# aleflabo/PREGO

Hardware: AMD Instinct MI355X
Metric: frames/sec (per-frame action logits) on Assembly101-O TSN features (higher is better)
Workload: dtype fp16; 1 GPU; BASELINE configs[1]: Assembly101-O-test-split-shaped eval set, MiniROAD eval path (rgb+flow fp32 [T,2048] each -> per-frame probs[86] + argmax); clips_per_gpu=182, frames_per_gpu=2306143, min_T=3342, max_T=33981, flow=non-zero (full K=4096 layer1 GEMM), parallelism=clip-sharded dp1, no collective: every rank its own eval-set-sized clip list, weights=random init, seed 20

## Files before the change

### prego_amd/csrc/ff_pass.hip

```cpp
#include "common.h"
#include "kernels.h"
#include "gemm_tile.h"
#include "pass_handshake.h"

#define FF_TIMEOUT_TICKS 200000000ull

__device__ __forceinline__ bool ffp_wait_ge(const unsigned* p, unsigned need, unsigned* abort_word, unsigned code) {
  if (__hip_atomic_load(p, __ATOMIC_RELAXED, __HIP_MEMORY_SCOPE_AGENT) >= need) return true;
  const unsigned long long t0 = __builtin_amdgcn_s_memrealtime();
  unsigned spins = 0;
  for (;;) {
    __builtin_amdgcn_s_sleep(8);
    if (__hip_atomic_load(p, __ATOMIC_RELAXED, __HIP_MEMORY_SCOPE_AGENT) >= need) return true;
    if ((++spins & 31u) == 0u) {
      if (__hip_atomic_load(abort_word, __ATOMIC_RELAXED, __HIP_MEMORY_SCOPE_AGENT)) return false;
      if (__builtin_amdgcn_s_memrealtime() - t0 > FF_TIMEOUT_TICKS) {
        __hip_atomic_store(abort_word, code, __ATOMIC_RELAXED, __HIP_MEMORY_SCOPE_AGENT);
        return false;
      }
    }
  }
}

template <typename OT, bool SC1OUT>
__device__ __forceinline__ void ffp_tile(char* smem, const bf16_t* __restrict__ A, int lda, int rows, const bf16_t* __restrict__ B, int ldb,
                                         const float* __restrict__ bias, bf16_t* __restrict__ C, int ldc, int K) {
  int tid = threadIdx.x;
  asm volatile("" : "+v"(tid));
  const int lane = tid & 63;
  const int wave = __builtin_amdgcn_readfirstlane(tid >> 6);
  const int grp = wave >> 2, wc = wave & 3;
  int a_off[2], b_off[2];
  pp_lane_offsets<false>(wave, lane, lda, ldb, 0, 0, a_off, b_off);
  const __amdgpu_buffer_rsrc_t rs_a = __builtin_amdgcn_make_buffer_rsrc((void*)A, 0, rows * lda * 2, 0x00020000);
  const __amdgpu_buffer_rsrc_t rs_b = __builtin_amdgcn_make_buffer_rsrc((void*)B, 0, 256 * ldb * 2, 0x00020000);
  const int fr = lane & 15, fq = lane >> 4;
  f32x4 acc[2][2][4][2];
#pragma unroll
  for (int x = 0; x < 2; ++x)
#pragma unroll
    for (int y = 0; y < 2; ++y)
#pragma unroll
      for (int i = 0; i < 4; ++i)
#pragma unroll
        for (int j = 0; j < 2; ++j) acc[x][y][i][j] = (f32x4){0.f, 0.f, 0.f, 0.f};
  pp_tile_loop<OT, false>((lds_char*)smem, rs_a, rs_b, a_off, b_off, lda, ldb, K / kPpBK, wave, lane, acc);
  float4 bv[2][2];
#pragma unroll
  for (int y = 0; y < 2; ++y)
#pragma unroll
    for (int j = 0; j < 2; ++j) bv[y][j] = *(const float4*)(bias + y * 128 + wc * 32 + fq * 8 + j * 4);
  const __amdgpu_buffer_rsrc_t rs_c = __builtin_amdgcn_make_buffer_rsrc((void*)C, 0, rows * ldc * 2, 0x00020000);
#pragma unroll
  for (int x = 0; x < 2; ++x)
#pragma unroll
    for (int y = 0; y < 2; ++y) {
      const int n = y * 128 + wc * 32 + fq * 8;
#pragma unroll
      for (int i = 0; i < 4; ++i) {
        const int m = x * 128 + grp * 64 + i * 16 + fr;
        const f32x4 v0 = acc[x][y][i][0], v1 = acc[x][y][i][1];
        u32x4 pk;
        pk[0] = op16<OT>::pack2_sat(v0[0] + bv[y][0].x, v0[1] + bv[y][0].y); pk[1] = op16<OT>::pack2_sat(v0[2] + bv[y][0].z, v0[3] + bv[y][0].w);
        pk[2] = op16<OT>::pack2_sat(v1[0] + bv[y][1].x, v1[1] + bv[y][1].y); pk[3] = op16<OT>::pack2_sat(v1[2] + bv[y][1].z, v1[3] + bv[y][1].w);
        if constexpr (SC1OUT) __builtin_amdgcn_raw_buffer_store_b128(pk, rs_c, (m * ldc + n) * 2, 0, AUX_SC1);
        else __builtin_amdgcn_raw_buffer_store_b128(pk, rs_c, (m * ldc + n) * 2, 0, 0);
      }
    }
}

template <typename OT, bool IN16>
__device__ __forceinline__ void ffp_pack_rows(const FfPassArgs& a, int my_rows, int wave, int lane, const char* srgb, const char* sflow,
                                              bf16_t* __restrict__ Xs) {
  constexpr int ES = IN16 ? 2 : 4, NV = IN16 ? 1 : 2;
  constexpr int PR = 2;
  const int din = a.kx;
  const int cr_rgb = (a.d_rgb + 2047) >> 11, cpr = cr_rgb + ((a.d_flow + 2047) >> 11);
  const int n_rounds = my_rows > 0 ? ((my_rows + PR - 1) / PR) * cpr : 0;
  auto readlane_ptr = [](const char* p, int l) -> const char* {
    const unsigned long long v = (unsigned long long)p;
    const unsigned lo = (unsigned)__builtin_amdgcn_readlane((int)(unsigned)v, l), hi = (unsigned)__builtin_amdgcn_readlane((int)(unsigned)(v >> 32), l);
// ... 287 lines not shown
#pragma unroll
      for (int e = 0; e < NR; ++e)
#pragma unroll
        for (int i = 0; i < MAXV; ++i)
          if (i < nv) raw[e][i] = nxt[e][i];
    }
  }
}

template <typename OT>
__device__ __forceinline__ void ffp_ln_any(const FfPassArgs& a, int nrows, const bf16_t* __restrict__ Ys, bf16_t* __restrict__ Es, const float* gb) {
  switch (a.E >> 9) {
    case 4: ffp_ln<OT, 4, 2>(a, nrows, Ys, Es, gb); break;
    case 2: ffp_ln<OT, 2, 4>(a, nrows, Ys, Es, gb); break;
    case 1: ffp_ln<OT, 1, 4>(a, nrows, Ys, Es, gb); break;
    default: ffp_ln_generic<OT, 8, 2>(a, nrows, Ys, Es); break;
  }
}

template <typename OT>
__global__ __launch_bounds__(512, 2) void ff_pass_kernel(FfPassArgs a) {
  extern __shared__ __attribute__((aligned(16))) char smem[];
  __shared__ int s_job[2];
  const int tid = threadIdx.x;
  const int xcc = __builtin_amdgcn_readfirstlane(__builtin_amdgcn_s_getreg((3 << 11) | 20) & 7);
  if (xcc < a.xcd_lo) return;
  if (tid == 0) {
    const unsigned nth = __hip_atomic_fetch_add(a.hs.ff_here + xcc, 1u, __ATOMIC_RELAXED, __HIP_MEMORY_SCOPE_AGENT);
    s_job[1] = hs_wait(a.hs, a.hs.ticks_all) == PREGO_HS_GO ? 1 : 0;
    if (a.max_wg > 0 && (int)nth >= a.max_wg) s_job[1] = 0;
  }
  __syncthreads();
  if (!__builtin_amdgcn_readfirstlane(s_job[1])) return;
  __shared__ __attribute__((aligned(16))) float s_gb[2 * FLN_MAX_E];
  if (a.E <= FLN_MAX_E)
    for (int c = tid; c < a.E; c += 512) { s_gb[c] = a.ln_g[c]; s_gb[FLN_MAX_E + c] = a.ln_b[c]; }
  const int q = xcc - a.xcd_lo, nf = 8 - a.xcd_lo;
  const int n_q = a.n_units > q ? (a.n_units - q + nf - 1) / nf : 0;
  const int sg = a.sg, tpr = sg * (2 + a.nt1 + a.nt2);
  const int n_rounds = (n_q + sg - 1) / sg + a.lag3;
  __shared__ unsigned long long s_stat[11];
  const bool stats = a.stats != nullptr && tid == 0;
  if (stats) {
    for (int e = 0; e < 8; ++e) s_stat[e] = 0;
    s_stat[9] = __builtin_amdgcn_s_memrealtime(); s_stat[8] = s_stat[9]; s_stat[10] = __builtin_amdgcn_s_memtime();
  }
#define FSTAT(i) do { if (stats) { const unsigned long long n_ = __builtin_amdgcn_s_memrealtime(); s_stat[i] += n_ - s_stat[8]; s_stat[8] = n_; } } while (0)
  for (;;) {
    __syncthreads();
    if (tid == 0) s_job[0] = (int)__hip_atomic_fetch_add(a.tick + q, 1u, __ATOMIC_RELAXED, __HIP_MEMORY_SCOPE_AGENT);
    __syncthreads();
    const int k = __builtin_amdgcn_readfirstlane(s_job[0]);
    const int round = k / tpr, j = k - round * tpr;
    FSTAT(5);
    if (round >= n_rounds) break;
    int type, i, nb = 0;
    if (j < sg) { type = 0; i = round * sg + j; }
    else if (j < sg + sg * a.nt1) { const int jj = j - sg; type = 1; nb = jj / sg; i = (round - a.lag1) * sg + (jj - nb * sg); }
    else if (j < 2 * sg + sg * a.nt1) { type = 2; i = (round - a.lag2) * sg + (j - sg - sg * a.nt1); }
    else { const int jj = j - 2 * sg - sg * a.nt1; type = 3; nb = jj / sg; i = (round - a.lag3) * sg + (jj - nb * sg); }
    if (i < 0 || i >= n_q) continue;
    const int u = q + i * nf;
    if (tid == 0) {
      bool ok = true;
      const int up = u - a.ring_units;
      if (type == 0) {
        if (up >= 0) ok = ffp_wait_ge(a.l1_cnt + up, (unsigned)a.nt1, a.abort_word, 0x100u);
      } else if (type == 1) {
        ok = ffp_wait_ge(a.pack_done + u, 1u, a.abort_word, 0x101u);
        if (ok && up >= 0) ok = ffp_wait_ge(a.ln_done + up, 1u, a.abort_word, 0x102u);
      } else if (type == 2) {
        ok = ffp_wait_ge(a.l1_cnt + u, (unsigned)a.nt1, a.abort_word, 0x103u);
        if (ok && up >= 0) ok = ffp_wait_ge(a.wih_cnt + up, (unsigned)a.nt2, a.abort_word, 0x104u);
      } else {
        ok = ffp_wait_ge(a.ln_done + u, 1u, a.abort_word, 0x105u);
        const int ug = u - a.gi_ring_units;
        if (ok && ug >= 0) ok = ffp_wait_ge(a.rec_cnt + (ug >> a.chunk_unit_shift), (unsigned)a.rec_expect, a.abort_word, 0x106u);
      }
      s_job[1] = ok ? 1 : 0;
    }
    __syncthreads();
    if (!__builtin_amdgcn_readfirstlane(s_job[1])) break;
    FSTAT(4);
    asm volatile("buffer_inv sc0" ::: "memory");
    const int row0 = u * 256;
    const int nrows = a.total_rows - row0 < 256 ? a.total_rows - row0 : 256;
    const size_t slot = (size_t)(u % a.ring_units) * 256;
    if (type == 0) {
      if (!(a.dbg & 1)) ffp_pack<OT>(a, row0, nrows, a.X + slot * a.kx);
    } else if (type == 1) {
      if (!(a.dbg & 4))
      ffp_tile<OT, false>(smem, a.X + slot * a.kx, a.kx, nrows, a.w1 + (size_t)nb * 256 * a.ld_w1, a.ld_w1, a.b1 + nb * 256,
                          a.Y + slot * a.E + nb * 256, a.E, a.kx);
    } else if (type == 2) {
      if (a.dbg & 2) { }
      else ffp_ln_any<OT>(a, nrows, a.Y + slot * a.E, a.Eb + slot * a.E, s_gb);
    } else {
      const size_t gslot = (size_t)(u & (a.gi_ring_units - 1)) * 256;
      if (!(a.dbg & 8))
      ffp_tile<OT, true>(smem, a.Eb + slot * a.E, a.E, nrows, a.w_ih + (size_t)nb * 256 * a.E, a.E, a.bias2 + nb * 256,
                         a.GI + gslot * a.n3 + nb * 256, a.n3, a.E);
    }
    asm volatile("s_waitcnt vmcnt(0)" ::: "memory");
    __syncthreads();
    FSTAT(type);
    if (tid == 0) {
      if (type == 0) __hip_atomic_store(a.pack_done + u, 1u, __ATOMIC_RELAXED, __HIP_MEMORY_SCOPE_AGENT);
      else if (type == 1) __hip_atomic_fetch_add(a.l1_cnt + u, 1u, __ATOMIC_RELAXED, __HIP_MEMORY_SCOPE_AGENT);
      else if (type == 2) __hip_atomic_store(a.ln_done + u, 1u, __ATOMIC_RELAXED, __HIP_MEMORY_SCOPE_AGENT);
      else {
        const unsigned old = __hip_atomic_fetch_add(a.wih_cnt + u, 1u, __ATOMIC_RELAXED, __HIP_MEMORY_SCOPE_AGENT);
        if (old + 1u == (unsigned)a.nt2)
          __hip_atomic_fetch_add(a.gi_cnt + (u >> a.chunk_unit_shift), 1u, __ATOMIC_RELAXED, __HIP_MEMORY_SCOPE_AGENT);
      }
    }
  }
  if (stats) {
    s_stat[7] = __builtin_amdgcn_s_memrealtime() - s_stat[9];
    s_stat[6] = __builtin_amdgcn_s_memtime() - s_stat[10];
    for (int e = 0; e < 8; ++e) atomicAdd(a.stats + e, s_stat[e]);
  }
#undef FSTAT
}

int launch_ff_pass(const FfPassArgs& a, hipStream_t s) {
  if (a.E % 512 || a.E > 4096 || a.kx % kPpBK || a.kx < 2 * kPpBK || a.n3 % 256 || a.xcd_lo < 1 || a.xcd_lo > 7) return -1;
  if (a.sg < 1 || a.ring_units % (8 - a.xcd_lo) || (a.gi_ring_units & (a.gi_ring_units - 1)) || a.nt1 != a.E / 256 || a.nt2 != a.n3 / 256) return -1;
  static DeviceOnce once;
  once.run([&] {
    (void)hipFuncSetAttribute((const void*)ff_pass_kernel<bf16_t>, hipFuncAttributeMaxDynamicSharedMemorySize, 2 * kPpBuf);
    (void)hipFuncSetAttribute((const void*)ff_pass_kernel<f16_t>, hipFuncAttributeMaxDynamicSharedMemorySize, 2 * kPpBuf);
  });
  if (a.f16) ff_pass_kernel<f16_t><<<256, 512, 2 * kPpBuf, s>>>(a);
  else ff_pass_kernel<bf16_t><<<256, 512, 2 * kPpBuf, s>>>(a);
  return 0;
}
```

### prego_amd/csrc/gemm_tile.h

```cpp
#pragma once
#include "common.h"
#include "kernels.h"
#include <type_traits>

template <typename F>
inline void gemm_epi_dispatch(int mode, bool f16, F&& f) {
  auto by_type = [&](auto e) { if (f16) f(e, f16_t{}); else f(e, bf16_t{}); };
  switch (mode) {
    case EPI_STORE: by_type(std::integral_constant<int, EPI_STORE>{}); break;
    case EPI_STORE_BF16: by_type(std::integral_constant<int, EPI_STORE_BF16>{}); break;
    case EPI_RESIDUAL: by_type(std::integral_constant<int, EPI_RESIDUAL>{}); break;
    case EPI_GELU_BF16: by_type(std::integral_constant<int, EPI_GELU_BF16>{}); break;
    case EPI_TOKENS: by_type(std::integral_constant<int, EPI_TOKENS>{}); break;
    default: by_type(std::integral_constant<int, EPI_QKV>{}); break;
  }
}

__device__ __forceinline__ int xcd_remap(int bid, int nwg) {
  const int q = nwg >> 3, r = nwg & 7, x = bid & 7;
  return (x < r ? x * (q + 1) : r * (q + 1) + (x - r) * q) + (bid >> 3);
}

__device__ __forceinline__ int tile_key_a(int r) { return (r >> 1) & 7; }
__device__ __forceinline__ int tile_key_b_perm(int r) { return ((r >> 1) & 1) | (((r >> 3) & 3) << 1); }
// ... 12 lines not shown
#pragma unroll
  for (int i = 0; i < 2; ++i) {
    const int r = (wave * 2 + i) * 8 + sr;
    const int c = scp ^ tile_key_a(r);
    const int cb = scp ^ tile_key_b_perm(r);
    if constexpr (SPLIT) {
      a_off[i] = r * lda * 2 + (c < 4 ? c * 16 : a_lo * 2 + (c - 4) * 16);
      b_off[i] = r * ldb * 2 + (cb < 4 ? cb * 16 : b_lo * 2 + (cb - 4) * 16);
    } else {
      a_off[i] = r * lda * 2 + c * 16;
      b_off[i] = r * ldb * 2 + cb * 16;
    }
  }
}

template <typename OT, bool SPLIT>
__device__ __forceinline__ void pp_tile_loop(lds_char* smem, __amdgpu_buffer_rsrc_t rs_a, __amdgpu_buffer_rsrc_t rs_b, const int (&a_off)[2],
                                             const int (&b_off)[2], int lda, int ldb, int nk, int wave, int lane, f32x4 (&acc)[2][2][4][2]) {
  const int grp = wave >> 2, wc = wave & 3;
  auto stage_a = [&](int hf, int kt) {
    lds_char* dst = smem + (kt & 1) * kPpBuf + hf * kPpHalf + wave * 2048;
    const int so = hf * 128 * lda * 2 + kt * (SPLIT ? kPpBK : kPpBK * 2);
#pragma unroll
    for (int i = 0; i < 2; ++i)
      __builtin_amdgcn_raw_ptr_buffer_load_lds(rs_a, (__attribute__((address_space(3))) void*)(dst + i * 1024), 16, a_off[i], so, 0, 0);
  };
  auto stage_b = [&](int hf, int kt) {
    lds_char* dst = smem + (kt & 1) * kPpBuf + (2 + hf) * kPpHalf + wave * 2048;
    const int so = hf * 128 * ldb * 2 + kt * (SPLIT ? kPpBK : kPpBK * 2);
#pragma unroll
    for (int i = 0; i < 2; ++i)
      __builtin_amdgcn_raw_ptr_buffer_load_lds(rs_b, (__attribute__((address_space(3))) void*)(dst + i * 1024), 16, b_off[i], so, 0, 0);
  };

  const int fr = lane & 15, fq = lane >> 4;
  bf16x8 a0[2][4], a1[2][4], b0[2][2], b1[2][2];
  auto read_a = [&](bf16x8 (&af)[2][4], int slot, int kt) {
    const lds_char* base = smem + (kt & 1) * kPpBuf + slot * kPpHalf;
#pragma unroll
    for (int ks = 0; ks < 2; ++ks)
#pragma unroll
      for (int i = 0; i < 4; ++i) {
        const int r = grp * 64 + fr;
        af[ks][i] = *(const lds_bf16x8*)(base + r * 128 + (((ks * 4 + fq) ^ tile_key_a(r)) << 4) + i * 2048);
      }
  };
  auto read_b = [&](bf16x8 (&bf)[2][2], int slot, int kt) {
    const lds_char* base = smem + (kt & 1) * kPpBuf + slot * kPpHalf;
// ... 26 lines not shown
      for (int ks = 0; ks < 2; ++ks)
#pragma unroll
        for (int i = 0; i < 4; ++i)
#pragma unroll
          for (int j = 0; j < 2; ++j) c[i][j] = op16<OT>::mfma(bf[ks][j], af[ks][i], c[i][j]);
    }
    __builtin_amdgcn_s_setprio(0);
    __builtin_amdgcn_sched_barrier(0);
  };
  auto bar = [&]() {
    __builtin_amdgcn_sched_barrier(0);
    __builtin_amdgcn_s_barrier();
    __builtin_amdgcn_sched_barrier(0);
  };

  stage_a(0, 0); stage_b(0, 0); stage_b(1, 0); stage_a(1, 0);
  stage_a(0, 1); stage_b(0, 1); stage_b(1, 1);
  GEMM_VMCNT(10);
  bar();
  read_a(a0, 0, 0);
  if (grp == 1) bar();
  for (int kt = 0; kt < nk; ++kt) {
    const bool full = kt + 2 < nk;
    read_b(b0, 2, kt);
    if (kt + 1 < nk) stage_a(1, kt + 1);
    if (full) GEMM_VMCNT(10); else GEMM_VMCNT(0);
    bar();
    mma(acc[0][0], a0, b0);
    bar();
    read_b(b1, 3, kt);
    if (full) { stage_a(0, kt + 2); GEMM_VMCNT(10); } else GEMM_VMCNT(0);
    bar();
// ... 88 lines not shown
```

### prego_amd/csrc/kernels.h

```cpp
#pragma once
#include <hip/hip_runtime_api.h>
#include <stddef.h>
#include <stdint.h>
#include <mutex>

const char* prego_tune_env(const char* name);

struct DeviceOnce {
  std::mutex mu;
  bool done[64] = {};
  template <class F> int run(F&& f) {
    int dev = 0;
    (void)hipGetDevice(&dev);
    if (dev < 0 || dev >= 64) { f(); return 0; }
    std::lock_guard<std::mutex> g(mu);
    if (!done[dev]) { f(); done[dev] = true; }
    return dev;
  }
};

#ifndef PREGO_HAVE_SLOTPLAN
struct SlotPlan {
  const int* rowoff; const int* nact; const int* seg_off; const int* seg_clip; const int* seg_start; const int* blk_step;
  int s_max; int n_slots;
// ... 59 lines not shown
  int E, n3;
  unsigned short* X; unsigned short* Y; unsigned short* Eb;
  unsigned short* GI;
  int ring_units, gi_ring_units;
  int total_rows, n_units;
  int xcd_lo;
  int chunk_unit_shift;
  int rec_expect;
  int nt1, nt2;
  int sg;
  int max_wg;
  int lag1, lag2, lag3;
  int dbg;
  unsigned long long* stats;
  int f16;
  unsigned* tick;
  unsigned* pack_done; unsigned* l1_cnt; unsigned* ln_done; unsigned* wih_cnt;
  unsigned* gi_cnt;
  const unsigned* rec_cnt;
  unsigned* abort_word;
  PassHandshake hs;
};
int launch_ff_pass(const FfPassArgs& a, hipStream_t s);
int launch_gru_recurrence_pass(int hid, GruArgs a, hipStream_t s);
int gru_group_size(bool bf16, int hid);
bool gru_hidden_supported(bool bf16, int hid);

struct GruArm { unsigned* hx; unsigned long long words_per_buf; unsigned pattern; unsigned* sync; };
GruArm gru_arm_desc(bool bf16, int hid, int G, void* hx, unsigned* sync);
void launch_gru_arm(const GruArm& arm, hipStream_t s);

// ... 402 lines not shown
```

### prego_amd/csrc/miniroad_split.cpp

```cpp
#include "miniroad_handle.h"

#include <algorithm>
#include <chrono>
#include <cstdlib>
#include <mutex>
#include <thread>

static int tuned_pow2(const char* name, int dflt) {
  const char* v = prego_tune_env(name);
  const int x = v ? atoi(v) : 0;
  return (x >= 16 && (x & (x - 1)) == 0) ? x : dflt;
}
static int split_gi_ring_units(int R) { return tuned_pow2("PREGO_SPLIT_GI_RING", R <= 3 ? 32 : 256); }
static const int kSplitRingPerXcd = (prego_tune_env("PREGO_SPLIT_RING_PER_XCD") && atoi(prego_tune_env("PREGO_SPLIT_RING_PER_XCD")) >= 12 &&
                                     atoi(prego_tune_env("PREGO_SPLIT_RING_PER_XCD")) % 4 == 0) ? atoi(prego_tune_env("PREGO_SPLIT_RING_PER_XCD")) : 24;
static const int kSplitSg = (prego_tune_env("PREGO_SPLIT_SG") && kSplitRingPerXcd % std::max(1, atoi(prego_tune_env("PREGO_SPLIT_SG"))) == 0)
                                ? std::max(1, atoi(prego_tune_env("PREGO_SPLIT_SG"))) : 2;
static int split_chunk_shift(int R) { return prego_tune_env("PREGO_SPLIT_CHUNK_SHIFT") ? atoi(prego_tune_env("PREGO_SPLIT_CHUNK_SHIFT")) : (R <= 3 ? 3 : 6); }
SplitRings split_rings(const prego_miniroad* h, int R) {
  SplitRings g;
  g.ring_units = kSplitRingPerXcd * (8 - R);
  g.x = align_up((size_t)g.ring_units * 256 * (size_t)(h->d_rgb + h->d_flow) * 2, 256);
  g.y = align_up((size_t)g.ring_units * 256 * (size_t)h->emb * 2, 256);
  g.e = g.y;
  g.gi = align_up((size_t)split_gi_ring_units(R) * 256 * (size_t)3 * h->hid * 2, 256);
  g.total = g.x + g.y + g.e + g.gi;
  return g;
}
bool split_workspace_ok(const prego_miniroad* h, int R, size_t workspace_bytes) { return workspace_bytes >= split_rings(h, R).total; }

size_t split_buf_need(const prego_miniroad* h, long long total) {
  const long long n_units = (total + 255) / 256;
  const int shift = split_chunk_shift(1);
// ... 28 lines not shown
  const int n_chunks = (n_units + upc - 1) >> chunk_shift;
  const SplitRings rg = split_rings(h, R);
  if (workspace_bytes < rg.total) return prego_fail_(PREGO_EWORKSPACE, "split pass: workspace %zu B < %zu B of rings", workspace_bytes, rg.total);
  char* wp = (char*)workspace;
  unsigned short* X = (unsigned short*)wp; wp += rg.x;
  unsigned short* Y = (unsigned short*)wp; wp += rg.y;
  unsigned short* Eb = (unsigned short*)wp; wp += rg.e;
  unsigned short* GI = (unsigned short*)wp;
  const size_t hr_bytes = align_up((size_t)total * H * 2, 256), rm_bytes = align_up((size_t)total * 8, 256);
  const size_t n_ctr = (size_t)4 * n_units + 2 * (size_t)n_chunks + 32;
  if (!h->chooser.split_warm) { h->chooser.meas_armed = false; h->chooser.split_warm = true; }
  if (!split_resident_ok(h, total)) return prego_fail_(PREGO_EWORKSPACE, "split pass: resident buffer %zu B < %zu B", h->res_bytes, split_buf_need(h, total));
  char* HR = h->res_buf;
  char* RM = HR + hr_bytes;
  unsigned* ctr = (unsigned*)(RM + rm_bytes);
  unsigned* tick = ctr; unsigned* hs_word = ctr + 8; unsigned* ff_here = ctr + 16; unsigned* pack_done = ctr + 32; unsigned* l1_cnt = pack_done + n_units; unsigned* ln_done = l1_cnt + n_units;
  unsigned* wih_cnt = ln_done + n_units; unsigned* gi_cnt = wih_cnt + n_units; unsigned* rec_cnt = gi_cnt + n_chunks;
  HIPCHK(hipMemsetAsync(ctr, 0, n_ctr * 4, s));
  HIPCHK(hipMemsetAsync(h->h_state, 0, (size_t)h->n_slots * H * 4, s));
  PassHandshake hs{};
  h->hs_seq = (h->hs_seq + 1u) & 0x3FFFFFFFu;
  if (h->hs_seq == 0u) h->hs_seq = 1u;
  hs.word = hs_word; hs.ff_here = ff_here; hs.host = h->pin_hs; hs.seq = h->hs_seq; hs.ticks_lead = 5000000u; hs.ticks_all = 10000000u;
  int fault = 0;
#ifdef PREGO_DEBUG_ABI
  fault = h->dbg_fault; h->dbg_fault = 0;
  if (fault == 3 || fault == 4) {
    HIPCHK(hipMemsetD32Async((hipDeviceptr_t)hs_word, PREGO_HS_GO, 1, s));
    HIPCHK(hipMemsetD32Async((hipDeviceptr_t)ff_here, 1, 8, s));
    if (fault == 3) HIPCHK(hipMemsetD32Async((hipDeviceptr_t)rec_cnt, R * h->P * 4, n_chunks, s));
    else HIPCHK(hipMemsetD32Async((hipDeviceptr_t)gi_cnt, upc, n_chunks, s));
// ... 4 lines not shown
  FfPassArgs fa{};
  fa.rgb_ptrs = tb.rgb; fa.flow_ptrs = with_flow ? tb.flow : nullptr; fa.plan = plan; fa.rowmap = RM;
  fa.d_rgb = h->d_rgb; fa.d_flow = with_flow ? h->d_flow : 0; fa.in16 = in16 ? 1 : 0; fa.kx = kx;
  fa.w1 = (const unsigned short*)h->w1; fa.ld_w1 = din; fa.b1 = h->b1; fa.ln_g = h->ln_g; fa.ln_b = h->ln_b; fa.ln_eps = 1e-5f;
  fa.w_ih = (const unsigned short*)h->w_ih_perm; fa.bias2 = h->bias2_perm; fa.E = E; fa.n3 = 3 * H;
  fa.X = X; fa.Y = Y; fa.Eb = Eb; fa.GI = GI; fa.ring_units = rg.ring_units; fa.gi_ring_units = gi_ring;
  fa.total_rows = total; fa.n_units = n_units; fa.xcd_lo = R; fa.chunk_unit_shift = chunk_shift;
  fa.rec_expect = R * h->P * 4; fa.nt1 = E / 256; fa.nt2 = 3 * H / 256;
  static const int lag1 = prego_tune_env("PREGO_SPLIT_LAG1") ? atoi(prego_tune_env("PREGO_SPLIT_LAG1")) : 2;
  static const int lag2 = prego_tune_env("PREGO_SPLIT_LAG2") ? atoi(prego_tune_env("PREGO_SPLIT_LAG2")) : 3;
  static const int lag3 = prego_tune_env("PREGO_SPLIT_LAG3") ? atoi(prego_tune_env("PREGO_SPLIT_LAG3")) : 4;
  static const bool want_stats = prego_tune_env("PREGO_SPLIT_STATS") != nullptr;
  fa.sg = kSplitSg; fa.lag1 = lag1; fa.lag2 = lag2; fa.lag3 = lag3; fa.f16 = h->f16 ? 1 : 0;
  static const int ff_cus = prego_tune_env("PREGO_SPLIT_FF_CUS") ? atoi(prego_tune_env("PREGO_SPLIT_FF_CUS")) : 0;
  fa.max_wg = ff_cus;
  fa.stats = want_stats ? h->stamps : nullptr;
#ifdef PREGO_DEBUG_ABI
  static const int dbg = prego_tune_env("PREGO_SPLIT_DBG") ? atoi(prego_tune_env("PREGO_SPLIT_DBG")) : 0;
  fa.dbg = dbg;
#endif
  fa.tick = tick; fa.pack_done = pack_done; fa.l1_cnt = l1_cnt; fa.ln_done = ln_done; fa.wih_cnt = wih_cnt; fa.gi_cnt = gi_cnt;
  fa.rec_cnt = rec_cnt; fa.abort_word = h->abort_word; fa.hs = hs;
  const int ring_sr = kSplitRingPerXcd / kSplitSg;
  if (lag1 < 1 || lag2 <= lag1 || lag3 <= lag2 || lag1 >= ring_sr || lag2 - ring_sr >= lag1 || lag3 - ring_sr >= lag2)
    return prego_fail_(PREGO_EINVAL, "split pass: lags %d %d %d", lag1, lag2, lag3);

  GruArgs ga{};
  ga.whh = h->w_hh; ga.b_hn = h->b_hn; ga.gi = GI; ga.gi_bf16 = 1; ga.f16 = h->f16 ? 1 : 0; ga.h_relu_out = HR; ga.h_raw_out = nullptr;
  ga.h_state = h->h_state; ga.hx = h->hx; ga.flags = h->flags; ga.abort_word = h->abort_word;
  ga.rowoff = h->d_rowoff; ga.nact = h->d_nact; ga.t0 = 0; ga.t1 = h->t_max; ga.row_base = 0; ga.rows = 0;
  ga.n_clips = h->n_slots; ga.G = h->G; ga.seg_off = h->plan_single ? nullptr : h->d_seg_off;
  ga.seg_start = h->plan_single ? nullptr : h->d_seg_start; ga.stamps = (h->use_stamps && !want_stats) ? h->stamps : nullptr;
  ga.sync = h->flags; ga.armed = 0; ga.Gd = R;
  ga.gi_cnt = gi_cnt; ga.rec_cnt = rec_cnt; ga.chunk_shift = chunk_shift + 8; ga.n_chunks = n_chunks;
  ga.units_per_chunk = upc; ga.units_last = n_units - upc * (n_chunks - 1); ga.gi_row_mask = (unsigned)gi_ring * 256u - 1u;
  ga.hs = hs;
// ... 78 lines not shown
```

Before: 25.22 million frames/s.

## Split FF pass workgroups into row and GEMM-tile workers with cross-tile prefetch

```diff
diff --git a/prego_amd/csrc/ff_pass.hip b/prego_amd/csrc/ff_pass.hip
--- a/prego_amd/csrc/ff_pass.hip
+++ b/prego_amd/csrc/ff_pass.hip
@@ -22,35 +22,38 @@
   }
 }
 
+struct FfpTile {
+  const bf16_t* A; const bf16_t* B; const float* bias; bf16_t* C;
+  int lda, ldb, ldc, K, rows;
+};
+__device__ __forceinline__ FfpTile ffp_tile_of(const FfPassArgs& a, int type, int nb, int u) {
+  FfpTile t;
+  const int row0 = u * 256;
+  t.rows = a.total_rows - row0 < 256 ? a.total_rows - row0 : 256;
+  const size_t slot = (size_t)(u % a.ring_units) * 256;
+  if (type == 1) {
+    t.A = a.X + slot * a.kx; t.lda = a.kx; t.B = a.w1 + (size_t)nb * 256 * a.ld_w1; t.ldb = a.ld_w1; t.bias = a.b1 + nb * 256;
+    t.C = a.Y + slot * a.E + nb * 256; t.ldc = a.E; t.K = a.kx;
+  } else {
+    const size_t gslot = (size_t)(u & (a.gi_ring_units - 1)) * 256;
+    t.A = a.Eb + slot * a.E; t.lda = a.E; t.B = a.w_ih + (size_t)nb * 256 * a.E; t.ldb = a.E; t.bias = a.bias2 + nb * 256;
+    t.C = a.GI + gslot * a.n3 + nb * 256; t.ldc = a.n3; t.K = a.E;
+  }
+  return t;
+}
+struct FfpOperands {
+  __amdgpu_buffer_rsrc_t rs_a, rs_b;
+  int a_off[2], b_off[2];
+};
+__device__ __forceinline__ void ffp_operands(const FfpTile& t, int wave, int lane, FfpOperands& o) {
+  pp_lane_offsets<false>(wave, lane, t.lda, t.ldb, 0, 0, o.a_off, o.b_off);
+  o.rs_a = __builtin_amdgcn_make_buffer_rsrc((void*)t.A, 0, t.rows * t.lda * 2, 0x00020000);
+  o.rs_b = __builtin_amdgcn_make_buffer_rsrc((void*)t.B, 0, 256 * t.ldb * 2, 0x00020000);
+}
 template <typename OT, bool SC1OUT>
-__device__ __forceinline__ void ffp_tile(char* smem, const bf16_t* __restrict__ A, int lda, int rows, const bf16_t* __restrict__ B, int ldb,
-                                         const float* __restrict__ bias, bf16_t* __restrict__ C, int ldc, int K) {
-  int tid = threadIdx.x;
-  asm volatile("" : "+v"(tid));
-  const int lane = tid & 63;
-  const int wave = __builtin_amdgcn_readfirstlane(tid >> 6);
-  const int grp = wave >> 2, wc = wave & 3;
-  int a_off[2], b_off[2];
-  pp_lane_offsets<false>(wave, lane, lda, ldb, 0, 0, a_off, b_off);
-  const __amdgpu_buffer_rsrc_t rs_a = __builtin_amdgcn_make_buffer_rsrc((void*)A, 0, rows * lda * 2, 0x00020000);
-  const __amdgpu_buffer_rsrc_t rs_b = __builtin_amdgcn_make_buffer_rsrc((void*)B, 0, 256 * ldb * 2, 0x00020000);
-  const int fr = lane & 15, fq = lane >> 4;
-  f32x4 acc[2][2][4][2];
-#pragma unroll
-  for (int x = 0; x < 2; ++x)
-#pragma unroll
-    for (int y = 0; y < 2; ++y)
-#pragma unroll
-      for (int i = 0; i < 4; ++i)
-#pragma unroll
-        for (int j = 0; j < 2; ++j) acc[x][y][i][j] = (f32x4){0.f, 0.f, 0.f, 0.f};
-  pp_tile_loop<OT, false>((lds_char*)smem, rs_a, rs_b, a_off, b_off, lda, ldb, K / kPpBK, wave, lane, acc);
-  float4 bv[2][2];
-#pragma unroll
-  for (int y = 0; y < 2; ++y)
-#pragma unroll
-    for (int j = 0; j < 2; ++j) bv[y][j] = *(const float4*)(bias + y * 128 + wc * 32 + fq * 8 + j * 4);
-  const __amdgpu_buffer_rsrc_t rs_c = __builtin_amdgcn_make_buffer_rsrc((void*)C, 0, rows * ldc * 2, 0x00020000);
+__device__ __forceinline__ void ffp_tile_store(const FfpTile& t, int wave, int lane, const f32x4 (&acc)[2][2][4][2], const float4 (&bv)[2][2]) {
+  const int grp = wave >> 2, wc = wave & 3, fr = lane & 15, fq = lane >> 4;
+  const __amdgpu_buffer_rsrc_t rs_c = __builtin_amdgcn_make_buffer_rsrc((void*)t.C, 0, t.rows * t.ldc * 2, 0x00020000);
 #pragma unroll
   for (int x = 0; x < 2; ++x)
 #pragma unroll
@@ -63,8 +66,8 @@
         u32x4 pk;
         pk[0] = op16<OT>::pack2_sat(v0[0] + bv[y][0].x, v0[1] + bv[y][0].y); pk[1] = op16<OT>::pack2_sat(v0[2] + bv[y][0].z, v0[3] + bv[y][0].w);
         pk[2] = op16<OT>::pack2_sat(v1[0] + bv[y][1].x, v1[1] + bv[y][1].y); pk[3] = op16<OT>::pack2_sat(v1[2] + bv[y][1].z, v1[3] + bv[y][1].w);
-        if constexpr (SC1OUT) __builtin_amdgcn_raw_buffer_store_b128(pk, rs_c, (m * ldc + n) * 2, 0, AUX_SC1);
-        else __builtin_amdgcn_raw_buffer_store_b128(pk, rs_c, (m * ldc + n) * 2, 0, 0);
+        if constexpr (SC1OUT) __builtin_amdgcn_raw_buffer_store_b128(pk, rs_c, (m * t.ldc + n) * 2, 0, AUX_SC1);
+        else __builtin_amdgcn_raw_buffer_store_b128(pk, rs_c, (m * t.ldc + n) * 2, 0, 0);
       }
     }
 }
@@ -382,7 +385,205 @@
     case 4: ffp_ln<OT, 4, 2>(a, nrows, Ys, Es, gb); break;
     case 2: ffp_ln<OT, 2, 4>(a, nrows, Ys, Es, gb); break;
     case 1: ffp_ln<OT, 1, 4>(a, nrows, Ys, Es, gb); break;
-    default: ffp_ln_generic<OT, 8, 2>(a, nrows, Ys, Es); break;
+    default: ffp_ln_generic<OT, 8, 1>(a, nrows, Ys, Es); break;
+  }
+}
+
+struct FfpQueue { int q, nf, n_q, n_rounds; };
+
+#define FSTAT(i) do { if (stats) { const unsigned long long n_ = __builtin_amdgcn_s_memrealtime(); s_stat[i] += n_ - s_stat[8]; s_stat[8] = n_; } } while (0)
+
+template <typename OT>
+__device__ __forceinline__ void ffp_row_worker(const FfPassArgs& a, const FfpQueue& g, int* s_job, const float* s_gb, unsigned long long* s_stat, bool stats) {
+  const int tid = threadIdx.x;
+  const int sg = a.sg, tpr = 2 * sg;
+  for (;;) {
+    __syncthreads();
+    if (tid == 0) s_job[0] = (int)__hip_atomic_fetch_add(a.tick + g.q, 1u, __ATOMIC_RELAXED, __HIP_MEMORY_SCOPE_AGENT);
+    __syncthreads();
+    const int k = __builtin_amdgcn_readfirstlane(s_job[0]);
+    const int round = k / tpr, j = k - round * tpr;
+    FSTAT(5);
+    if (round >= g.n_rounds) break;
+    int type, i;
+    if (j < sg) { type = 0; i = round * sg + j; }
+    else { type = 2; i = (round - a.lag2) * sg + (j - sg); }
+    if (i < 0 || i >= g.n_q) continue;
+    const int u = g.q + i * g.nf;
+    if (tid == 0) {
+      bool ok = true;
+      const int up = u - a.ring_units;
+      if (type == 0) {
+        if (up >= 0) ok = ffp_wait_ge(a.l1_cnt + up, (unsigned)a.nt1, a.abort_word, 0x100u);
+      } else {
+        ok = ffp_wait_ge(a.l1_cnt + u, (unsigned)a.nt1, a.abort_word, 0x103u);
+        if (ok && up >= 0) ok = ffp_wait_ge(a.wih_cnt + up, (unsigned)a.nt2, a.abort_word, 0x104u);
+      }
+      s_job[1] = ok ? 1 : 0;
+    }
+    __syncthreads();
+    if (!__builtin_amdgcn_readfirstlane(s_job[1])) break;
+    FSTAT(4);
+    asm volatile("buffer_inv sc0" ::: "memory");
+    const int row0 = u * 256;
+    const int nrows = a.total_rows - row0 < 256 ? a.total_rows - row0 : 256;
+    const size_t slot = (size_t)(u % a.ring_units) * 256;
+    if (type == 0) {
+      if (!(a.dbg & 1)) ffp_pack<OT>(a, row0, nrows, a.X + slot * a.kx);
+    } else {
+      if (!(a.dbg & 2)) ffp_ln_any<OT>(a, nrows, a.Y + slot * a.E, a.Eb + slot * a.E, s_gb);
+    }
+    asm volatile("s_waitcnt vmcnt(0)" ::: "memory");
+    __syncthreads();
+    FSTAT(type);
+    if (tid == 0) {
+      if (type == 0) __hip_atomic_store(a.pack_done + u, 1u, __ATOMIC_RELAXED, __HIP_MEMORY_SCOPE_AGENT);
+      else __hip_atomic_store(a.ln_done + u, 1u, __ATOMIC_RELAXED, __HIP_MEMORY_SCOPE_AGENT);
+    }
+  }
+}
+
+__device__ __forceinline__ int ffp_tile_ticket(const FfPassArgs& a, const FfpQueue& g, int k, int& type, int& nb, int& u) {
+  const int sg = a.sg, tpr = sg * (a.nt1 + a.nt2);
+  const int round = k / tpr, j = k - round * tpr;
+  type = 1; nb = 0; u = 0;
+  if (round >= g.n_rounds) return 2;
+  int i;
+  if (j < sg * a.nt1) { nb = j / sg; i = (round - a.lag1) * sg + (j - nb * sg); }
+  else { const int jj = j - sg * a.nt1; type = 3; nb = jj / sg; i = (round - a.lag3) * sg + (jj - nb * sg); }
+  if (i < 0 || i >= g.n_q) return 1;
+  u = g.q + i * g.nf;
+  return 0;
+}
+__device__ __forceinline__ bool ffp_tile_wait(const FfPassArgs& a, int type, int u) {
+  bool ok;
+  if (type == 1) {
+    const int up = u - a.ring_units;
+    ok = ffp_wait_ge(a.pack_done + u, 1u, a.abort_word, 0x101u);
+    if (ok && up >= 0) ok = ffp_wait_ge(a.ln_done + up, 1u, a.abort_word, 0x102u);
+  } else {
+    const int ug = u - a.gi_ring_units;
+    ok = ffp_wait_ge(a.ln_done + u, 1u, a.abort_word, 0x105u);
+    if (ok && ug >= 0) ok = ffp_wait_ge(a.rec_cnt + (ug >> a.chunk_unit_shift), (unsigned)a.rec_expect, a.abort_word, 0x106u);
+  }
+  return ok;
+}
+__device__ __forceinline__ bool ffp_tile_ready(const FfPassArgs& a, int type, int u) {
+  const unsigned* p0; const unsigned* p1; unsigned n1;
+  if (type == 1) {
+    const int up = u - a.ring_units;
+    p0 = a.pack_done + u; p1 = up >= 0 ? a.ln_done + up : p0; n1 = up >= 0 ? 1u : 0u;
+  } else {
+    const int ug = u - a.gi_ring_units;
+    p0 = a.ln_done + u; p1 = ug >= 0 ? a.rec_cnt + (ug >> a.chunk_unit_shift) : p0; n1 = ug >= 0 ? (unsigned)a.rec_expect : 0u;
+  }
+  const unsigned v0 = __hip_atomic_load(p0, __ATOMIC_RELAXED, __HIP_MEMORY_SCOPE_AGENT);
+  const unsigned v1 = __hip_atomic_load(p1, __ATOMIC_RELAXED, __HIP_MEMORY_SCOPE_AGENT);
+  return v0 >= 1u && v1 >= n1;
+}
+
+template <typename OT>
+__device__ __forceinline__ void ffp_tile_worker(const FfPassArgs& a, const FfpQueue& g, char* smem, int* s_job, unsigned long long* s_stat, bool stats) {
+  const int tid = threadIdx.x;
+  unsigned* tk = a.tick_tile + g.q;
+  auto first_tile = [&](int k) -> int {
+    for (;;) {
+      int ty, nb, u;
+      const int st = ffp_tile_ticket(a, g, k, ty, nb, u);
+      if (st == 0) return k;
+      if (st == 2) return -1;
+      k = __builtin_amdgcn_readfirstlane((int)__hip_atomic_fetch_add(tk, 1u, __ATOMIC_RELAXED, __HIP_MEMORY_SCOPE_AGENT));
+    }
+  };
+  __syncthreads();
+  if (tid == 0) s_job[0] = first_tile(__builtin_amdgcn_readfirstlane((int)__hip_atomic_fetch_add(tk, 1u, __ATOMIC_RELAXED, __HIP_MEMORY_SCOPE_AGENT)));
+  __syncthreads();
+  int k = __builtin_amdgcn_readfirstlane(s_job[0]);
+  FSTAT(5);
+  bool staged = false;
+  unsigned nk = 0;
+  if (tid == 0 && k >= 0) nk = __hip_atomic_fetch_add(tk, 1u, __ATOMIC_RELAXED, __HIP_MEMORY_SCOPE_AGENT);
+  while (k >= 0) {
+    int type, nb, u;
+    (void)ffp_tile_ticket(a, g, k, type, nb, u);
+    if (!staged) {
+      if (tid == 0) s_job[1] = ffp_tile_wait(a, type, u) ? 1 : 0;
+      __syncthreads();
+      if (!__builtin_amdgcn_readfirstlane(s_job[1])) break;
+      FSTAT(4);
+      asm volatile("buffer_inv sc0" ::: "memory");
+    }
+    const FfpTile t = ffp_tile_of(a, type, nb, u);
+    const bool skip = (a.dbg & (type == 1 ? 4 : 8)) != 0;
+    int tid_ = threadIdx.x;
+    asm volatile("" : "+v"(tid_));
+    const int lane = tid_ & 63;
+    const int wave = __builtin_amdgcn_readfirstlane(tid_ >> 6);
+    f32x4 acc[2][2][4][2];
+#pragma unroll
+    for (int x = 0; x < 2; ++x)
+#pragma unroll
+      for (int y = 0; y < 2; ++y)
+#pragma unroll
+        for (int i = 0; i < 4; ++i)
+#pragma unroll
+          for (int j = 0; j < 2; ++j) acc[x][y][i][j] = (f32x4){0.f, 0.f, 0.f, 0.f};
+    if (!skip) {
+      FfpOperands o;
+      ffp_operands(t, wave, lane, o);
+      pp_tile_loop<OT, false, true>((lds_char*)smem, o.rs_a, o.rs_b, o.a_off, o.b_off, t.lda, t.ldb, t.K / kPpBK, wave, lane, acc, staged);
+    } else {
+      __syncthreads();
+    }
+    const int wc = wave & 3, fq = lane >> 4;
+    float4 bv[2][2];
+#pragma unroll
+    for (int y = 0; y < 2; ++y)
+#pragma unroll
+      for (int j = 0; j < 2; ++j) bv[y][j] = *(const float4*)(t.bias + y * 128 + wc * 32 + fq * 8 + j * 4);
+    if (tid == 0) {
+      const int kn = first_tile(__builtin_amdgcn_readfirstlane((int)nk));
+      int go = 0;
+      if (kn >= 0 && !(a.dbg & 12)) {
+        int ty, nb2, u2;
+        (void)ffp_tile_ticket(a, g, kn, ty, nb2, u2);
+        go = ffp_tile_ready(a, ty, u2) ? 1 : 0;
+      }
+      s_job[0] = kn; s_job[1] = go;
+      if (kn >= 0) nk = __hip_atomic_fetch_add(tk, 1u, __ATOMIC_RELAXED, __HIP_MEMORY_SCOPE_AGENT);
+    }
+#pragma unroll
+    for (int y = 0; y < 2; ++y)
+#pragma unroll
+      for (int j = 0; j < 2; ++j) asm volatile("" : "+v"(bv[y][j].x), "+v"(bv[y][j].y), "+v"(bv[y][j].z), "+v"(bv[y][j].w));
+    __syncthreads();
+    const int kn = __builtin_amdgcn_readfirstlane(s_job[0]);
+    const bool go = __builtin_amdgcn_readfirstlane(s_job[1]) != 0;
+    if (go) {
+      asm volatile("buffer_inv sc0" ::: "memory");
+      int ty, nb2, u2;
+      (void)ffp_tile_ticket(a, g, kn, ty, nb2, u2);
+      const FfpTile t2 = ffp_tile_of(a, ty, nb2, u2);
+      FfpOperands o2;
+      ffp_operands(t2, wave, lane, o2);
+      pp_tile_prologue<false>((lds_char*)smem, o2.rs_a, o2.rs_b, o2.a_off, o2.b_off, t2.lda, t2.ldb, wave);
+    }
+    if (!skip) {
+      if (type == 3) ffp_tile_store<OT, true>(t, wave, lane, acc, bv);
+      else ffp_tile_store<OT, false>(t, wave, lane, acc, bv);
+    }
+    asm volatile("s_waitcnt vmcnt(0)" ::: "memory");
+    __syncthreads();
+    FSTAT(type);
+    if (tid == 0) {
+      if (type == 1) __hip_atomic_fetch_add(a.l1_cnt + u, 1u, __ATOMIC_RELAXED, __HIP_MEMORY_SCOPE_AGENT);
+      else {
+        const unsigned old = __hip_atomic_fetch_add(a.wih_cnt + u, 1u, __ATOMIC_RELAXED, __HIP_MEMORY_SCOPE_AGENT);
+        if (old + 1u == (unsigned)a.nt2)
+          __hip_atomic_fetch_add(a.gi_cnt + (u >> a.chunk_unit_shift), 1u, __ATOMIC_RELAXED, __HIP_MEMORY_SCOPE_AGENT);
+      }
+    }
+    k = kn; staged = go;
   }
 }
 
@@ -395,105 +596,46 @@
   if (xcc < a.xcd_lo) return;
   if (tid == 0) {
     const unsigned nth = __hip_atomic_fetch_add(a.hs.ff_here + xcc, 1u, __ATOMIC_RELAXED, __HIP_MEMORY_SCOPE_AGENT);
+    s_job[0] = (int)(nth & 31u);
     s_job[1] = hs_wait(a.hs, a.hs.ticks_all) == PREGO_HS_GO ? 1 : 0;
     if (a.max_wg > 0 && (int)nth >= a.max_wg) s_job[1] = 0;
   }
   __syncthreads();
   if (!__builtin_amdgcn_readfirstlane(s_job[1])) return;
+  const bool row = __builtin_amdgcn_readfirstlane(s_job[0]) < a.row_wgs;
   __shared__ __attribute__((aligned(16))) float s_gb[2 * FLN_MAX_E];
-  if (a.E <= FLN_MAX_E)
+  if (row && a.E <= FLN_MAX_E)
     for (int c = tid; c < a.E; c += 512) { s_gb[c] = a.ln_g[c]; s_gb[FLN_MAX_E + c] = a.ln_b[c]; }
-  const int q = xcc - a.xcd_lo, nf = 8 - a.xcd_lo;
-  const int n_q = a.n_units > q ? (a.n_units - q + nf - 1) / nf : 0;
-  const int sg = a.sg, tpr = sg * (2 + a.nt1 + a.nt2);
-  const int n_rounds = (n_q + sg - 1) / sg + a.lag3;
+  FfpQueue g;
+  g.q = xcc - a.xcd_lo; g.nf = 8 - a.xcd_lo;
+  g.n_q = a.n_units > g.q ? (a.n_units - g.q + g.nf - 1) / g.nf : 0;
+  g.n_rounds = (g.n_q + a.sg - 1) / a.sg + a.lag3;
   __shared__ unsigned long long s_stat[11];
   const bool stats = a.stats != nullptr && tid == 0;
   if (stats) {
     for (int e = 0; e < 8; ++e) s_stat[e] = 0;
     s_stat[9] = __builtin_amdgcn_s_memrealtime(); s_stat[8] = s_stat[9]; s_stat[10] = __builtin_amdgcn_s_memtime();
   }
-#define FSTAT(i) do { if (stats) { const unsigned long long n_ = __builtin_amdgcn_s_memrealtime(); s_stat[i] += n_ - s_stat[8]; s_stat[8] = n_; } } while (0)
-  for (;;) {
-    __syncthreads();
-    if (tid == 0) s_job[0] = (int)__hip_atomic_fetch_add(a.tick + q, 1u, __ATOMIC_RELAXED, __HIP_MEMORY_SCOPE_AGENT);
-    __syncthreads();
-    const int k = __builtin_amdgcn_readfirstlane(s_job[0]);
-    const int round = k / tpr, j = k - round * tpr;
-    FSTAT(5);
-    if (round >= n_rounds) break;
-    int type, i, nb = 0;
-    if (j < sg) { type = 0; i = round * sg + j; }
-    else if (j < sg + sg * a.nt1) { const int jj = j - sg; type = 1; nb = jj / sg; i = (round - a.lag1) * sg + (jj - nb * sg); }
-    else if (j < 2 * sg + sg * a.nt1) { type = 2; i = (round - a.lag2) * sg + (j - sg - sg * a.nt1); }
-    else { const int jj = j - 2 * sg - sg * a.nt1; type = 3; nb = jj / sg; i = (round - a.lag3) * sg + (jj - nb * sg); }
-    if (i < 0 || i >= n_q) continue;
-    const int u = q + i * nf;
-    if (tid == 0) {
-      bool ok = true;
-      const int up = u - a.ring_units;
-      if (type == 0) {
-        if (up >= 0) ok = ffp_wait_ge(a.l1_cnt + up, (unsigned)a.nt1, a.abort_word, 0x100u);
-      } else if (type == 1) {
-        ok = ffp_wait_ge(a.pack_done + u, 1u, a.abort_word, 0x101u);
-        if (ok && up >= 0) ok = ffp_wait_ge(a.ln_done + up, 1u, a.abort_word, 0x102u);
-      } else if (type == 2) {
-        ok = ffp_wait_ge(a.l1_cnt + u, (unsigned)a.nt1, a.abort_word, 0x103u);
-        if (ok && up >= 0) ok = ffp_wait_ge(a.wih_cnt + up, (unsigned)a.nt2, a.abort_word, 0x104u);
-      } else {
-        ok = ffp_wait_ge(a.ln_done + u, 1u, a.abort_word, 0x105u);
-        const int ug = u - a.gi_ring_units;
-        if (ok && ug >= 0) ok = ffp_wait_ge(a.rec_cnt + (ug >> a.chunk_unit_shift), (unsigned)a.rec_expect, a.abort_word, 0x106u);
-      }
-      s_job[1] = ok ? 1 : 0;
-    }
-    __syncthreads();
-    if (!__builtin_amdgcn_readfirstlane(s_job[1])) break;
-    FSTAT(4);
-    asm volatile("buffer_inv sc0" ::: "memory");
-    const int row0 = u * 256;
-    const int nrows = a.total_rows - row0 < 256 ? a.total_rows - row0 : 256;
-    const size_t slot = (size_t)(u % a.ring_units) * 256;
-    if (type == 0) {
-      if (!(a.dbg & 1)) ffp_pack<OT>(a, row0, nrows, a.X + slot * a.kx);
-    } else if (type == 1) {
-      if (!(a.dbg & 4))
-      ffp_tile<OT, false>(smem, a.X + slot * a.kx, a.kx, nrows, a.w1 + (size_t)nb * 256 * a.ld_w1, a.ld_w1, a.b1 + nb * 256,
-                          a.Y + slot * a.E + nb * 256, a.E, a.kx);
-    } else if (type == 2) {
-      if (a.dbg & 2) { }
-      else ffp_ln_any<OT>(a, nrows, a.Y + slot * a.E, a.Eb + slot * a.E, s_gb);
-    } else {
-      const size_t gslot = (size_t)(u & (a.gi_ring_units - 1)) * 256;
-      if (!(a.dbg & 8))
-      ffp_tile<OT, true>(smem, a.Eb + slot * a.E, a.E, nrows, a.w_ih + (size_t)nb * 256 * a.E, a.E, a.bias2 + nb * 256,
-                         a.GI + gslot * a.n3 + nb * 256, a.n3, a.E);
-    }
-    asm volatile("s_waitcnt vmcnt(0)" ::: "memory");
-    __syncthreads();
-    FSTAT(type);
-    if (tid == 0) {
-      if (type == 0) __hip_atomic_store(a.pack_done + u, 1u, __ATOMIC_RELAXED, __HIP_MEMORY_SCOPE_AGENT);
-      else if (type == 1) __hip_atomic_fetch_add(a.l1_cnt + u, 1u, __ATOMIC_RELAXED, __HIP_MEMORY_SCOPE_AGENT);
-      else if (type == 2) __hip_atomic_store(a.ln_done + u, 1u, __ATOMIC_RELAXED, __HIP_MEMORY_SCOPE_AGENT);
-      else {
-        const unsigned old = __hip_atomic_fetch_add(a.wih_cnt + u, 1u, __ATOMIC_RELAXED, __HIP_MEMORY_SCOPE_AGENT);
-        if (old + 1u == (unsigned)a.nt2)
-          __hip_atomic_fetch_add(a.gi_cnt + (u >> a.chunk_unit_shift), 1u, __ATOMIC_RELAXED, __HIP_MEMORY_SCOPE_AGENT);
-      }
-    }
-  }
-  if (stats) {
+  auto flush = [&]() {
+    if (!stats) return;
     s_stat[7] = __builtin_amdgcn_s_memrealtime() - s_stat[9];
     s_stat[6] = __builtin_amdgcn_s_memtime() - s_stat[10];
     for (int e = 0; e < 8; ++e) atomicAdd(a.stats + e, s_stat[e]);
-  }
+  };
+  if (!row) {
+    ffp_tile_worker<OT>(a, g, smem, s_job, s_stat, stats);
+    flush();
+    return;
+  }
+  ffp_row_worker<OT>(a, g, s_job, s_gb, s_stat, stats);
+  flush();
+}
 #undef FSTAT
-}
 
 int launch_ff_pass(const FfPassArgs& a, hipStream_t s) {
   if (a.E % 512 || a.E > 4096 || a.kx % kPpBK || a.kx < 2 * kPpBK || a.n3 % 256 || a.xcd_lo < 1 || a.xcd_lo > 7) return -1;
   if (a.sg < 1 || a.ring_units % (8 - a.xcd_lo) || (a.gi_ring_units & (a.gi_ring_units - 1)) || a.nt1 != a.E / 256 || a.nt2 != a.n3 / 256) return -1;
+  if (a.row_wgs < 1 || a.row_wgs > 31 || (a.max_wg > 0 && (a.max_wg > 32 || a.max_wg <= a.row_wgs)) || !a.tick || !a.tick_tile) return -1;
   static DeviceOnce once;
   once.run([&] {
     (void)hipFuncSetAttribute((const void*)ff_pass_kernel<bf16_t>, hipFuncAttributeMaxDynamicSharedMemorySize, 2 * kPpBuf);
diff --git a/prego_amd/csrc/gemm_tile.h b/prego_amd/csrc/gemm_tile.h
--- a/prego_amd/csrc/gemm_tile.h
+++ b/prego_amd/csrc/gemm_tile.h
@@ -50,24 +50,38 @@
   }
 }
 
-template <typename OT, bool SPLIT>
+template <bool SPLIT>
+__device__ __forceinline__ void pp_stage_a(lds_char* smem, __amdgpu_buffer_rsrc_t rs_a, const int (&a_off)[2], int lda, int wave, int hf, int kt) {
+  lds_char* dst = smem + (kt & 1) * kPpBuf + hf * kPpHalf + wave * 2048;
+  const int so = hf * 128 * lda * 2 + kt * (SPLIT ? kPpBK : kPpBK * 2);
+#pragma unroll
+  for (int i = 0; i < 2; ++i)
+    __builtin_amdgcn_raw_ptr_buffer_load_lds(rs_a, (__attribute__((address_space(3))) void*)(dst + i * 1024), 16, a_off[i], so, 0, 0);
+}
+template <bool SPLIT>
+__device__ __forceinline__ void pp_stage_b(lds_char* smem, __amdgpu_buffer_rsrc_t rs_b, const int (&b_off)[2], int ldb, int wave, int hf, int kt) {
+  lds_char* dst = smem + (kt & 1) * kPpBuf + (2 + hf) * kPpHalf + wave * 2048;
+  const int so = hf * 128 * ldb * 2 + kt * (SPLIT ? kPpBK : kPpBK * 2);
+#pragma unroll
+  for (int i = 0; i < 2; ++i)
+    __builtin_amdgcn_raw_ptr_buffer_load_lds(rs_b, (__attribute__((address_space(3))) void*)(dst + i * 1024), 16, b_off[i], so, 0, 0);
+}
+template <bool SPLIT>
+__device__ __forceinline__ void pp_tile_prologue(lds_char* smem, __amdgpu_buffer_rsrc_t rs_a, __amdgpu_buffer_rsrc_t rs_b, const int (&a_off)[2],
+                                                 const int (&b_off)[2], int lda, int ldb, int wave) {
+  pp_stage_a<SPLIT>(smem, rs_a, a_off, lda, wave, 0, 0); pp_stage_b<SPLIT>(smem, rs_b, b_off, ldb, wave, 0, 0);
+  pp_stage_b<SPLIT>(smem, rs_b, b_off, ldb, wave, 1, 0); pp_stage_a<SPLIT>(smem, rs_a, a_off, lda, wave, 1, 0);
+  pp_stage_a<SPLIT>(smem, rs_a, a_off, lda, wave, 0, 1); pp_stage_b<SPLIT>(smem, rs_b, b_off, ldb, wave, 0, 1);
+  pp_stage_b<SPLIT>(smem, rs_b, b_off, ldb, wave, 1, 1);
+}
+
+template <typename OT, bool SPLIT, bool EXT = false>
 __device__ __forceinline__ void pp_tile_loop(lds_char* smem, __amdgpu_buffer_rsrc_t rs_a, __amdgpu_buffer_rsrc_t rs_b, const int (&a_off)[2],
-                                             const int (&b_off)[2], int lda, int ldb, int nk, int wave, int lane, f32x4 (&acc)[2][2][4][2]) {
+                                             const int (&b_off)[2], int lda, int ldb, int nk, int wave, int lane, f32x4 (&acc)[2][2][4][2],
+                                             bool staged = false) {
   const int grp = wave >> 2, wc = wave & 3;
-  auto stage_a = [&](int hf, int kt) {
-    lds_char* dst = smem + (kt & 1) * kPpBuf + hf * kPpHalf + wave * 2048;
-    const int so = hf * 128 * lda * 2 + kt * (SPLIT ? kPpBK : kPpBK * 2);
-#pragma unroll
-    for (int i = 0; i < 2; ++i)
-      __builtin_amdgcn_raw_ptr_buffer_load_lds(rs_a, (__attribute__((address_space(3))) void*)(dst + i * 1024), 16, a_off[i], so, 0, 0);
-  };
-  auto stage_b = [&](int hf, int kt) {
-    lds_char* dst = smem + (kt & 1) * kPpBuf + (2 + hf) * kPpHalf + wave * 2048;
-    const int so = hf * 128 * ldb * 2 + kt * (SPLIT ? kPpBK : kPpBK * 2);
-#pragma unroll
-    for (int i = 0; i < 2; ++i)
-      __builtin_amdgcn_raw_ptr_buffer_load_lds(rs_b, (__attribute__((address_space(3))) void*)(dst + i * 1024), 16, b_off[i], so, 0, 0);
-  };
+  auto stage_a = [&](int hf, int kt) { pp_stage_a<SPLIT>(smem, rs_a, a_off, lda, wave, hf, kt); };
+  auto stage_b = [&](int hf, int kt) { pp_stage_b<SPLIT>(smem, rs_b, b_off, ldb, wave, hf, kt); };
 
   const int fr = lane & 15, fq = lane >> 4;
   bf16x8 a0[2][4], a1[2][4], b0[2][2], b1[2][2];
@@ -124,8 +138,7 @@
     __builtin_amdgcn_sched_barrier(0);
   };
 
-  stage_a(0, 0); stage_b(0, 0); stage_b(1, 0); stage_a(1, 0);
-  stage_a(0, 1); stage_b(0, 1); stage_b(1, 1);
+  if (!(EXT && staged)) pp_tile_prologue<SPLIT>(smem, rs_a, rs_b, a_off, b_off, lda, ldb, wave);
   GEMM_VMCNT(10);
   bar();
   read_a(a0, 0, 0);
diff --git a/prego_amd/csrc/kernels.h b/prego_amd/csrc/kernels.h
--- a/prego_amd/csrc/kernels.h
+++ b/prego_amd/csrc/kernels.h
@@ -97,7 +97,9 @@
   int dbg;
   unsigned long long* stats;
   int f16;
+  int row_wgs;
   unsigned* tick;
+  unsigned* tick_tile;
   unsigned* pack_done; unsigned* l1_cnt; unsigned* ln_done; unsigned* wih_cnt;
   unsigned* gi_cnt;
   const unsigned* rec_cnt;
diff --git a/prego_amd/csrc/miniroad_split.cpp b/prego_amd/csrc/miniroad_split.cpp
--- a/prego_amd/csrc/miniroad_split.cpp
+++ b/prego_amd/csrc/miniroad_split.cpp
@@ -17,6 +17,12 @@
 static const int kSplitSg = (prego_tune_env("PREGO_SPLIT_SG") && kSplitRingPerXcd % std::max(1, atoi(prego_tune_env("PREGO_SPLIT_SG"))) == 0)
                                 ? std::max(1, atoi(prego_tune_env("PREGO_SPLIT_SG"))) : 2;
 static int split_chunk_shift(int R) { return prego_tune_env("PREGO_SPLIT_CHUNK_SHIFT") ? atoi(prego_tune_env("PREGO_SPLIT_CHUNK_SHIFT")) : (R <= 3 ? 3 : 6); }
+static int split_row_wgs(int R) {
+  const char* v = prego_tune_env("PREGO_SPLIT_ROW_WGS");
+  const int x = v ? atoi(v) : 0;
+  if (x >= 1 && x <= 31) return x;
+  return R <= 3 ? 5 : 5;
+}
 SplitRings split_rings(const prego_miniroad* h, int R) {
   SplitRings g;
   g.ring_units = kSplitRingPerXcd * (8 - R);
@@ -75,7 +81,7 @@
   char* HR = h->res_buf;
   char* RM = HR + hr_bytes;
   unsigned* ctr = (unsigned*)(RM + rm_bytes);
-  unsigned* tick = ctr; unsigned* hs_word = ctr + 8; unsigned* ff_here = ctr + 16; unsigned* pack_done = ctr + 32; unsigned* l1_cnt = pack_done + n_units; unsigned* ln_done = l1_cnt + n_units;
+  unsigned* tick = ctr; unsigned* hs_word = ctr + 8; unsigned* ff_here = ctr + 16; unsigned* tick_tile = ctr + 24; unsigned* pack_done = ctr + 32; unsigned* l1_cnt = pack_done + n_units; unsigned* ln_done = l1_cnt + n_units;
   unsigned* wih_cnt = ln_done + n_units; unsigned* gi_cnt = wih_cnt + n_units; unsigned* rec_cnt = gi_cnt + n_chunks;
   HIPCHK(hipMemsetAsync(ctr, 0, n_ctr * 4, s));
   HIPCHK(hipMemsetAsync(h->h_state, 0, (size_t)h->n_slots * H * 4, s));
@@ -110,12 +116,17 @@
   fa.sg = kSplitSg; fa.lag1 = lag1; fa.lag2 = lag2; fa.lag3 = lag3; fa.f16 = h->f16 ? 1 : 0;
   static const int ff_cus = prego_tune_env("PREGO_SPLIT_FF_CUS") ? atoi(prego_tune_env("PREGO_SPLIT_FF_CUS")) : 0;
   fa.max_wg = ff_cus;
+  fa.row_wgs = split_row_wgs(R);
+  if (ff_cus > 0) {
+    if (ff_cus < 2 || ff_cus > 32) return prego_fail_(PREGO_EINVAL, "split pass: PREGO_SPLIT_FF_CUS %d (2 .. 32: a row and a tile worker)", ff_cus);
+    fa.row_wgs = std::min(fa.row_wgs, ff_cus - 1);
+  }
   fa.stats = want_stats ? h->stamps : nullptr;
 #ifdef PREGO_DEBUG_ABI
   static const int dbg = prego_tune_env("PREGO_SPLIT_DBG") ? atoi(prego_tune_env("PREGO_SPLIT_DBG")) : 0;
   fa.dbg = dbg;
 #endif
-  fa.tick = tick; fa.pack_done = pack_done; fa.l1_cnt = l1_cnt; fa.ln_done = ln_done; fa.wih_cnt = wih_cnt; fa.gi_cnt = gi_cnt;
+  fa.tick = tick; fa.tick_tile = tick_tile; fa.pack_done = pack_done; fa.l1_cnt = l1_cnt; fa.ln_done = ln_done; fa.wih_cnt = wih_cnt; fa.gi_cnt = gi_cnt;
   fa.rec_cnt = rec_cnt; fa.abort_word = h->abort_word; fa.hs = hs;
   const int ring_sr = kSplitRingPerXcd / kSplitSg;
   if (lag1 < 1 || lag2 <= lag1 || lag3 <= lag2 || lag1 >= ring_sr || lag2 - ring_sr >= lag1 || lag3 - ring_sr >= lag2)
```

Result: slower. 24.51 million frames/s (-2.8%).
